# gcorso/DiffDock

Measured on NVIDIA H100. Metric: poses/sec at 20 diffusion steps, higher is better.
Workload: dtype f32

## Files before the change

diffdock_b200/cg_model.py:

```python
from __future__ import annotations

import math
import os

import numpy as np
import torch
from torch import nn

from . import ops
from .irreps import irreps_str, sh_irreps
from .hetero import receptor_blocks
from .layers import (AtomEncoder, GaussianSmearing, _mlp, check_confidence_widths, check_forward, confidence_head, cross_cutoff,
                     cross_graph, edge_cutoff, edge_weight, ligand_graph, score_heads)
from .synthetic import LIG_FEATURE_DIMS as lig_feature_dims, REC_RESIDUE_FEATURE_DIMS as rec_residue_feature_dims
from .tensor_layers import TensorProductConvLayer, get_irrep_seq
from .tp_table import full_tensor_product

_TABLES = os.path.join(os.path.dirname(os.path.abspath(__file__)), 'tables', 'score_norm_tables.npz')
SO3_MIN_EPS, SO3_MAX_EPS, SO3_N_EPS = 0.0005, 4, 2000
TORUS_SIGMA_MIN, TORUS_SIGMA_MAX, TORUS_SIGMA_N = 3e-3, 2, 5000


def _i32(t):
    return t.to(torch.int32).contiguous()
# ... 49 lines not shown
        super().__init__()
        assert parallel == 1, "not implemented"
        unsupported = dict(separate_noise_schedule=separate_noise_schedule,
                           asyncronous_noise_schedule=asyncronous_noise_schedule,
                           include_miscellaneous_atoms=include_miscellaneous_atoms, sidechain_pred=sidechain_pred,
                           depthwise_convolution=depthwise_convolution)
        bad = [k for k, v in unsupported.items() if v]
        if bad:
            raise NotImplementedError(f"{bad}: outside the hot path built so far (SURVEY.md section 8)")
        if lm_embedding_type not in (None, 'precomputed'):
            raise NotImplementedError("on-the-fly ESM embeddings are preprocessing (out of scope); use 'precomputed'")
        self.t_to_sigma, self.device, self.timestep_emb_func = t_to_sigma, device, timestep_emb_func
        self.in_lig_edge_features, self.sigma_embed_dim = in_lig_edge_features, sigma_embed_dim
        self.lig_max_radius, self.rec_max_radius = lig_max_radius, rec_max_radius
        self.cross_max_distance, self.dynamic_max_cross = cross_max_distance, dynamic_max_cross
        self.center_max_distance = center_max_distance
        self.distance_embed_dim, self.cross_distance_embed_dim = distance_embed_dim, cross_distance_embed_dim
        self.sh_lmax = sh_lmax
        self.sh_irreps = irreps_str(sh_irreps(sh_lmax))
        self.ns, self.nv = ns, nv
        self.scale_by_sigma, self.norm_by_sigma = scale_by_sigma, norm_by_sigma
        self.no_torsion, self.smooth_edges, self.odd_parity = no_torsion, smooth_edges, odd_parity
        self.confidence_mode, self.affinity_prediction = confidence_mode, affinity_prediction
        self.atom_confidence, self.atom_num_confidence_outputs = atom_confidence, atom_num_confidence_outputs
        self.num_conv_layers, self.num_prot_emb_layers = num_conv_layers, num_prot_emb_layers
        self.fixed_center_conv, self.no_aminoacid_identities = fixed_center_conv, no_aminoacid_identities
        self.differentiate_convolutions, self.reduce_pseudoscalars = differentiate_convolutions, reduce_pseudoscalars
        self.embed_also_ligand = embed_also_ligand
        self.lm_embedding_type = lm_embedding_type
        lm_dim = 1280 if lm_embedding_type == 'precomputed' else 0
        S, D, Dx = sigma_embed_dim, distance_embed_dim, cross_distance_embed_dim

        self.lig_node_embedding = AtomEncoder(emb_dim=ns, feature_dims=lig_feature_dims, sigma_embed_dim=S)
        self.lig_edge_embedding = _mlp(in_lig_edge_features + S + D, ns, ns, dropout)
        self.rec_node_embedding = AtomEncoder(emb_dim=ns, feature_dims=rec_residue_feature_dims, sigma_embed_dim=0,
                                              lm_embedding_dim=lm_dim)
        self.rec_edge_embedding = _mlp(D, ns, ns, dropout)
        self.rec_sigma_embedding = _mlp(S, ns, ns, dropout)
        self.cross_edge_embedding = _mlp(S + Dx, ns, ns, dropout)
        self.lig_distance_expansion = GaussianSmearing(0.0, lig_max_radius, D)
        self.rec_distance_expansion = GaussianSmearing(0.0, rec_max_radius, D)
        self.cross_distance_expansion = GaussianSmearing(0.0, cross_max_distance, Dx)

        self._irrep_seq = get_irrep_seq(ns, nv, use_second_order_repr, reduce_pseudoscalars)
        self._conv_kw = dict(sh_irreps=self.sh_irreps, n_edge_features=3 * ns, hidden_features=3 * ns, residual=True,
                             batch_norm=batch_norm, dropout=dropout, faster=sh_lmax == 1 and not use_second_order_repr,
                             tp_weights_layers=tp_weights_layers)
        self.rec_emb_layers = nn.ModuleList([self.conv(i, 1) for i in range(num_prot_emb_layers)])
        if embed_also_ligand:
            self.lig_emb_layers = nn.ModuleList([self.conv(i, 1) for i in range(num_prot_emb_layers)])
        self.conv_layers = self._interaction_stack(4, 2)
        self._sync_free = None
        self._prune_receptor = True
        if confidence_mode:
            self._confidence_heads(confidence_dropout, confidence_no_batchnorm, num_confidence_outputs)
            return

        self.center_distance_expansion = GaussianSmearing(0.0, center_max_distance, D)
        self.center_edge_embedding = _mlp(D + S, ns, ns, dropout)
        self.final_conv = TensorProductConvLayer(in_irreps=self.conv_layers[-1].out_irreps, sh_irreps=self.sh_irreps,
                                                 out_irreps='2x1o + 2x1e' if not odd_parity else '1x1o + 1x1e',
                                                 n_edge_features=2 * ns, residual=False, dropout=dropout,
                                                 batch_norm=batch_norm)
        self.tr_final_layer = nn.Sequential(nn.Linear(1 + S, ns), nn.Dropout(dropout), nn.ReLU(), nn.Linear(ns, 1))
        self.rot_final_layer = nn.Sequential(nn.Linear(1 + S, ns), nn.Dropout(dropout), nn.ReLU(), nn.Linear(ns, 1))
        if not no_torsion:
            self.final_edge_embedding = _mlp(D, ns, ns, dropout)
            T, tor_sh = full_tensor_product(self.sh_irreps, '1x2e')
            self.register_buffer('_tor_tp', torch.from_numpy(T).float(), persistent=False)
            self.tor_bond_conv = TensorProductConvLayer(in_irreps=self.conv_layers[-1].out_irreps,
                                                        sh_irreps=irreps_str(tor_sh),
                                                        out_irreps=f'{ns}x0o + {ns}x0e' if not odd_parity else f'{ns}x0o',
                                                        n_edge_features=3 * ns, residual=False, dropout=dropout,
                                                        batch_norm=batch_norm)
            self.tor_final_layer = nn.Sequential(nn.Linear(2 * ns if not odd_parity else ns, ns, bias=False), nn.Tanh(),
                                                 nn.Dropout(dropout), nn.Linear(ns, 1, bias=False))
        z = np.load(_TABLES)
        self.register_buffer('_so3_table', torch.from_numpy(z['so3_exp_score_norms']).float(), persistent=False)
        self.register_buffer('_torus_table', torch.from_numpy(z['torus_score_norm']).float(), persistent=False)

    def _confidence_heads(self, dropout, no_batchnorm, num_confidence_outputs):
        ns = self.ns
        self._conf_tail = (self.nv if self.reduce_pseudoscalars else ns) \
            if self.num_conv_layers + self.num_prot_emb_layers >= 3 else 0
        n_in = ns + self._conf_tail

        def head(i, o):
            bn = (lambda: nn.Identity()) if no_batchnorm else (lambda: nn.BatchNorm1d(ns))
            return nn.Sequential(nn.Linear(i, ns), bn(), nn.ReLU(), nn.Dropout(dropout), nn.Linear(ns, ns), bn(), nn.ReLU(),
                                 nn.Dropout(dropout), nn.Linear(ns, o))
        if self.atom_confidence:
            self.atom_confidence_predictor = head(n_in, self.atom_num_confidence_outputs + ns)
            n_in = ns
        self.confidence_predictor = head(n_in, num_confidence_outputs + (1 if self.affinity_prediction else 0))
        check_confidence_widths(self)

    def conv(self, i, groups):
        seq = self._irrep_seq
        return TensorProductConvLayer(in_irreps=seq[min(i, len(seq) - 1)], out_irreps=seq[min(i + 1, len(seq) - 1)],
                                      edge_groups=groups, **self._conv_kw)

    def _interaction_stack(self, groups, last_groups):
        P, L = self.num_prot_emb_layers, self.num_conv_layers
        return nn.ModuleList([self.conv(i, 1 if not self.differentiate_convolutions else
                                        (last_groups if i == P + L - 1 else groups)) for i in range(P, P + L)])

# ... 105 lines not shown

    def sync_free_crop_capable(self):
        return self.sync_free_capable() and all(layer.fused_capable(self.ns, self.ns) for layer in self.rec_emb_layers)

    @torch.no_grad()
    def forward(self, data):
        check_forward(self, data)
        c = self._static(data)
        if self.sync_free_capable() and max(c['rec_max'], c.get('atom_max', 0)) <= 10000:
            return self._forward_sync_free(data, c)
        if getattr(data, '_crop', None) is not None:
            raise RuntimeError("per-step receptor cropping (data._crop) runs on the sync-free forward only, which this "
                               "batch cannot take (more than 10000 residues in a complex)")
        return self._forward_host_sized(data, c)

    def _interaction_layers(self, node, groups, n_last, merge=False, shared=None, per_layer=None):
        L = len(self.conv_layers)
        for l, layer in enumerate(self.conv_layers):
            use, init = (groups if l < L - 1 else groups[:n_last]), None
            if per_layer is not None and per_layer[1][l] is not None:
                k = per_layer[0]
                use = use[:k] + [per_layer[1][l]] + use[k + 1:]
            if l == 0 and shared is not None:
                init, skip = shared
                use = use[:skip] + [None] + use[skip + 1:]
            if merge:
                use = [tuple(torch.cat([g[k] for g in use]) if use[0][k] is not None else None for k in range(5))]
            node = layer.forward_groups(node, use, gather_scalars=self.ns, init=init)
        return node

    def _forward_sync_free(self, data, c):
        lig, rec = data['ligand'], data['receptor']
        ns, n_lig = self.ns, lig.batch.shape[0]
        tr_sigma, rot_sigma, tor_sigma = self._sigmas(data)

        sig = self.rec_sigma_embedding(self.timestep_emb_func(data.complex_t['tr'])).contiguous()
        crop = getattr(data, '_crop', None)
        prune = self._prune_receptor and len(self.conv_layers) > 1
        keep = None
        if crop is None:
            rec_node, rec_pos = rec.rec_node_attr.clone(), rec.pos.float().contiguous()
            rr_tgt32 = _rr_joint(c, n_lig)
            g_rr = (rr_tgt32[0], rr_tgt32[1], c['rr_ea'], c['rr_vec'], _flat(c['rr_ew']),
                    dict(ea_add=sig, ea_add_idx=c['rr_gid32']))
        else:
            rec_node, rec_pos, g_rr, keep = self._cropped_receptor(data, c, crop, sig, n_lig, select=not prune)
        rec_node[:, :ns] += sig[rec.batch]
        lig_node, g_ll = self._ligand_graph_sync_free(data, c)

        r, rpg = cross_cutoff(self, tr_sigma)
        g_lr, g_rl = self._cross_graph_sync_free(data, c, rec_pos, c['rec_ptr'], c['rec_batch32'],
                                                 c['rec_max'], c['cap_cross'], r, rpg, n_lig, self.cross_edge_embedding,
                                                 self.cross_distance_expansion, vec_sign=-1.0)

        node = torch.cat([lig_node, rec_node], 0)
        groups = [g_ll,
                  g_lr,
                  g_rr,
                  g_rl]
        shared = self._shared_receptor_messages(data, c, rec, rec_node, sig, n_lig) \
            if len(self.conv_layers) > 1 and crop is None else None
        pruned = self._pruned_contact_groups(c, g_rl, keep, sig, n_lig, rec_node.shape[0], shared is not None) \
            if prune else None
        node = self._interaction_layers(node, groups, 2, shared=(shared, 2) if shared is not None else None,
                                        per_layer=(2, pruned) if pruned is not None else None)
        return self._heads(data, c, node[:n_lig], tr_sigma, rot_sigma, tor_sigma, sync_free=True)

    def _need_levels(self, L, shared):
        return [None if l == L - 1 or (l == 0 and shared) else L - 1 - l for l in range(L)]

    def _pruned_contact_groups(self, c, g_rl, keep, sig, n_lig, n_rec, shared):
        levels = self._need_levels(len(self.conv_layers), shared)
        n_levels = max((k for k in levels if k is not None), default=0)
        if n_levels == 0:
            return None
        if 'rr_tgt32l' not in c:
            c['rr_tgt32l'] = (_i32(c['rr_tgt']), _i32(c['rr_src']))
        tgt32, src32 = c['rr_tgt32l']
        key = ('prune', n_lig, n_levels)
        if key not in c:
            c[key] = (torch.empty((n_levels, n_rec), dtype=torch.uint8, device=tgt32.device),
                      [ops.select_edges_buffers(tgt32.shape[0], tgt32.device) for _ in range(n_levels)])
        need_buf, bufs = c[key]
        need = ops.receptor_need(g_rl[0], g_rl[5]['n_edges_dev'], n_lig, tgt32, src32, n_rec, n_levels, keep=keep,
                                 out=need_buf)
        ew, sel = _flat(c['rr_ew']), {}
        for k in sorted({k for k in levels if k is not None}):
            t, s_, perm, gid, n_dev = ops.crop_select_edges(tgt32, src32, keep, c['rr_gid32'], offset=n_lig,
                                                            need=need[k - 1], out=bufs[k - 1])
            sel[k] = (t, s_, c['rr_ea'], c['rr_vec'], ew,
                      dict(n_edges_dev=n_dev, edge_perm=perm, ea_add=sig, ea_add_idx=gid))
        return [sel[k] if k is not None else None for k in levels]

    def _cropped_receptor(self, data, c, crop, sig, n_lig, select=True):
        if not self.sync_free_crop_capable():
            raise RuntimeError("per-step receptor cropping needs every receptor embedding layer on the fused kernel "
                               "(CGModel.sync_free_crop_capable)")
        lig, rec = data['ligand'], data['receptor']
        keep, rec_pos = ops.crop_flags(lig.pos.float().contiguous(), c['lig_ptr'], rec.pos.float().contiguous(),
                                       c['rec_batch32'], crop[0], crop[1])
        if 'rr_tgt32l' not in c:
            c['rr_tgt32l'] = (_i32(c['rr_tgt']), _i32(c['rr_src']))
        if not select and not len(self.rec_emb_layers):
            return rec.rec_node_attr.clone(), rec_pos, None, keep
        tgt, src, perm, gid, n_dev = ops.crop_select_edges(*c['rr_tgt32l'], keep, c['rr_gid32'], offset=n_lig)
        ew = _flat(c['rr_ew'])
# ... 155 lines not shown
```

diffdock_b200/csrc/fused_conv.cu:

```cuda
#include <cuda_bf16.h>
#include <cuda_runtime.h>
#include <stdint.h>
#include <stdlib.h>

#include "../../include/diffdock_b200.h"
#include "sm90.cuh"

namespace {

using namespace ddb200_sm90;

constexpr int BM = 64, BK = 64;
constexpr int CTA_EDGES = 2 * BM;
constexpr int A_KB_BYTES = BM * BK * 2;
constexpr int B_IMAGE_BYTES = 256 * BK * 2;
constexpr int MAX_N = 192;
constexpr int STAGES = 4;
constexpr int STAGE_BYTES = MAX_N * BK * 2;
constexpr int MAX_KB = 5;
constexpr int MAX_KA = MAX_KB;
constexpr int A_IMAGE_BYTES = MAX_KA * A_KB_BYTES;
constexpr int OPS_PER_KB = 8;
constexpr int THREADS = 256;
constexpr int MAX_TILES = 128, MAX_PATHS = 16, MTAB = 48;
constexpr int BAR_WG = 1;
constexpr int SO_STAGES = 3, SO_MAX_PATHS = 32, SO_MTAB = 128;

__device__ __forceinline__ void red_add(float* addr, float v) {
  asm volatile("red.global.add.f32 [%0], %1;" ::"l"(addr), "f"(v) : "memory");
}
__device__ __forceinline__ void wgmma_wait_one() { asm volatile("wgmma.wait_group.sync.aligned 1;" ::: "memory"); }

__device__ __forceinline__ void put_a(unsigned char* sA, int r, int col, __nv_bfloat16 v) {
  const int kb = col >> 6, c = (col & 63) >> 3, j = col & 7;
  *reinterpret_cast<__nv_bfloat16*>(sA + (size_t)kb * A_KB_BYTES + r * 128 + ((c ^ (r & 7)) << 4) + j * 2) = v;
}
__device__ __forceinline__ void put_a2(unsigned char* sA, int r, int col, uint32_t v) {
  const int kb = col >> 6, c = (col & 63) >> 3, j = col & 7;
  *reinterpret_cast<uint32_t*>(sA + (size_t)kb * A_KB_BYTES + r * 128 + ((c ^ (r & 7)) << 4) + j * 2) = v;
}
__device__ __forceinline__ void put_a8(unsigned char* sA, int r, int col0, const uint4& v) {
  const int kb = col0 >> 6, c = (col0 & 63) >> 3;
  *reinterpret_cast<uint4*>(sA + (size_t)kb * A_KB_BYTES + r * 128 + ((c ^ (r & 7)) << 4)) = v;
}
__device__ __forceinline__ void split1(float f, __nv_bfloat16& hi, __nv_bfloat16& lo) {
  hi = __float2bfloat16(f);
  lo = __float2bfloat16(f - __bfloat162float(hi));
}
__device__ __forceinline__ void split8(const float* f, uint4& hi, uint4& lo) {
  uint32_t h[4], l[4];
#pragma unroll
  for (int i = 0; i < 4; ++i) {
    __nv_bfloat16 h0, h1, l0, l1;
    split1(f[2 * i], h0, l0);
    split1(f[2 * i + 1], h1, l1);
    h[i] = (uint32_t)__bfloat16_as_ushort(h0) | ((uint32_t)__bfloat16_as_ushort(h1) << 16);
    l[i] = (uint32_t)__bfloat16_as_ushort(l0) | ((uint32_t)__bfloat16_as_ushort(l1) << 16);
  }
  hi = make_uint4(h[0], h[1], h[2], h[3]);
// ... 651 lines not shown
      atomicAdd(p.dbg + 14, dwait[1]);
      dwait[0] = dwait[1] = 0ull;
    }
  }
  if (p.dbg && blockIdx.x == 0 && tid == 0) {
    unsigned long long g1;
    asm volatile("mov.u64 %0, %%globaltimer;" : "=l"(g1));
    atomicAdd(p.dbg + 25, (unsigned long long)clock64());
    atomicAdd(p.dbg + 26, g1);
  }
}

__global__ void __launch_bounds__(THREADS, 1) fused_conv_kernel(const FusedParams p) { fused_conv_body<false>(p); }
__global__ void __launch_bounds__(THREADS, 1) fused_conv_kernel_so(const FusedParams p) { fused_conv_body<true>(p); }

constexpr int MAX_DEVICES = 64;
struct DeviceState {
  bool attr_done = false, attr_done_so = false;
  bool dbg_init = false;
  unsigned long long* dbg = nullptr;
};
DeviceState g_dev[MAX_DEVICES];

unsigned long long* fused_debug_buffer(int dev) {
  if (dev < 0 || dev >= MAX_DEVICES) return nullptr;
  DeviceState& st = g_dev[dev];
  if (!st.dbg_init) {
    st.dbg_init = true;
    const char* e = getenv("DDB200_FUSED_DEBUG");
    if (e && atoi(e) != 0 && cudaMalloc(&st.dbg, 32 * sizeof(unsigned long long)) == cudaSuccess)
      cudaMemset(st.dbg, 0, 32 * sizeof(unsigned long long));
  }
  return st.dbg;
}

}


extern "C" int ddb200_fused_debug_read(uint64_t* out) {
  int dev = 0;
  cudaGetDevice(&dev);
  unsigned long long* b = fused_debug_buffer(dev);
  if (!b || !out) return DDB200_EINVAL;
  cudaError_t e = cudaDeviceSynchronize();
  if (e == cudaSuccess) e = cudaMemcpy(out, b, 32 * sizeof(unsigned long long), cudaMemcpyDeviceToHost);
  if (e == cudaSuccess) e = cudaMemset(b, 0, 32 * sizeof(unsigned long long));
  return (int)e;
}

namespace {

template <bool SO>
int fused_conv_launch(const ddb200_fused_args* a, void* stream) {
  if (!a || !a->edge_attr || !a->w1_images || !a->w2_images || !a->tiles || !a->mtab || !a->x || !a->edge_vec || !a->sum ||
      !a->tgt || !a->src || a->n_edges < 0 || a->ne <= 0 || a->ns < 0 || a->hidden <= 0 || a->n_tiles <= 0 || a->d_out <= 0)
    return DDB200_EINVAL;
  if (a->ns > 0 && (!a->node || a->ld_node < a->ns)) return DDB200_EINVAL;
  if (a->n_tiles > MAX_TILES || a->n_paths <= 0 || a->n_paths > (SO ? SO_MAX_PATHS : MAX_PATHS) || a->sh_lmax < 0 ||
      a->sh_lmax > 2)
    return DDB200_EINVAL;
  if ((a->ea_add == nullptr) != (a->ea_add_idx == nullptr)) return DDB200_EINVAL;
  const int K1 = a->ne + 2 * a->ns, H = a->hidden;
  const int K1p = (K1 + 15) / 16 * 16, Hp = (H + 15) / 16 * 16;
  const int n_kb = (2 * Hp + 16 + BK - 1) / BK, n_kb1 = (2 * K1p + 16 + BK - 1) / BK;
  if (n_kb > MAX_KB || n_kb1 > MAX_KB || H > MAX_N) return DDB200_EINVAL;
  if ((reinterpret_cast<uintptr_t>(a->w1_images) & 127) || (reinterpret_cast<uintptr_t>(a->w2_images) & 127)) return DDB200_EINVAL;
  if (a->n_hidden < 0 || (a->n_hidden > 0 && (!a->wh_images || (reinterpret_cast<uintptr_t>(a->wh_images) & 127))))
    return DDB200_EINVAL;
  if (a->n_edges == 0) return 0;
  FusedParams p = {};
  p.ea = a->edge_attr; p.ld_ea = a->ld_ea; p.ne = a->ne; p.node = a->node; p.ld_node = a->ld_node; p.ns = a->ns;
  p.tgt = a->tgt; p.src = a->src; p.perm = a->edge_perm; p.ea_add = a->ea_add; p.ea_add_idx = a->ea_add_idx;
  const auto al16 = [](const void* q) { return (reinterpret_cast<uintptr_t>(q) & 15) == 0; };
  p.a0_vec = ((a->ne | a->ns) & 7) == 0 && ((a->ld_ea | (a->ns ? a->ld_node : 0)) & 3) == 0 && al16(a->edge_attr) &&
             (a->ns == 0 || al16(a->node)) && (a->ea_add == nullptr || al16(a->ea_add));
  p.vec_sign = a->vec_sign == 0.f ? 1.f : a->vec_sign;
  p.w1img = reinterpret_cast<const __nv_bfloat16*>(a->w1_images); p.K1 = K1; p.K1p = K1p; p.n_kb1 = n_kb1;
  p.H = H; p.Hp = Hp; p.n_kb = n_kb;
  p.w2img = reinterpret_cast<const __nv_bfloat16*>(a->w2_images); p.tiles = a->tiles; p.n_tiles = a->n_tiles;
  p.whimg = reinterpret_cast<const __nv_bfloat16*>(a->wh_images); p.n_hidden = a->n_hidden;
  p.mtab = a->mtab; p.n_paths = a->n_paths;
  p.x = a->x; p.ld_x = a->ld_x; p.x_vec2 = (a->x_pairs_ok && (a->ld_x & 1) == 0 && (reinterpret_cast<uintptr_t>(a->x) & 7) == 0) ? 1 : 0;
  p.vec = a->edge_vec; p.ew = a->edge_weight; p.lmax = a->sh_lmax; p.sum = a->sum; p.d_out = a->d_out; p.cnt = a->cnt;
  p.n_edges = a->n_edges; p.n_edges_dev = a->n_edges_dev;
  int dev = 0, sms = 132;
  cudaGetDevice(&dev);
  if (dev < 0 || dev >= MAX_DEVICES) return DDB200_EINVAL;
  p.dbg = fused_debug_buffer(dev);
  cudaDeviceGetAttribute(&sms, cudaDevAttrMultiProcessorCount, dev);
  const long long n_mtiles = (a->n_edges + CTA_EDGES - 1) / CTA_EDGES;
  const size_t smem = smem_bytes<SO>();
  if (smem > 227 * 1024) return DDB200_ESMEM;
  auto kernel = SO ? fused_conv_kernel_so : fused_conv_kernel;
  bool& attr_done = SO ? g_dev[dev].attr_done_so : g_dev[dev].attr_done;
  if (!attr_done) {
    const cudaError_t e = cudaFuncSetAttribute(kernel, cudaFuncAttributeMaxDynamicSharedMemorySize, (int)smem);
    if (e != cudaSuccess) return (int)e;
    attr_done = true;
  }
  const unsigned grid = (unsigned)(n_mtiles < sms ? n_mtiles : sms);
  kernel<<<grid, THREADS, smem, (cudaStream_t)stream>>>(p);
  return (int)cudaGetLastError();
}

}

extern "C" int ddb200_fused_conv(const ddb200_fused_args* a, void* stream) { return fused_conv_launch<false>(a, stream); }
// ... 3 lines not shown
```

diffdock_b200/fused.py:

```python
from __future__ import annotations

import ctypes as C
import os

import numpy as np
import torch

from . import _lib
from .ops import PROFILE, _need_cuda, _ptr, _stream

from .irreps import real_cg
from .radial import BK, BN
from .tp_table import TpTable

CONSUMER_KINDS = {(48, 1): (0, 4), (10, 3): (1, 16), (16, 1): (2, 8), (4, 3): (3, 16), (10, 1): (4, 16), (4, 1): (5, 16),
                  (10, 5): (6, 16), (4, 5): (7, 16)}
MAX_K = 144
MAX_TILES = 128
MTAB = 48
MAX_PATHS = 16
MTAB_SO = 128
MAX_PATHS_SO = 32
ENABLED = os.environ.get('DDB200_FUSED_CONV', '1') != '0'

# ... 52 lines not shown
        self.n_hidden = len(hidden)
        self.second_order = second_order(table)
        paths = sorted(table.paths, key=lambda p: (p.i_out, p.w_ref_off))
        tiles, row_src = [], []
        D = 5 if self.second_order else 3
        mtab = np.zeros((len(paths), MTAB_SO if self.second_order else MTAB), dtype=np.float32)
        for pi, p in enumerate(paths):
            C = real_cg(p.l_in, p.l_sh, p.l_out)
            d_in, d_sh, d_out = C.shape
            blk = np.zeros((D, D, 5))
            blk[:d_in, :d_out, :d_sh] = p.coef * np.transpose(C, (0, 2, 1))
            mtab[pi, :D * D * 5] = blk.reshape(-1)
        group_prev = None
        path_prev = None
        for pi, p in enumerate(paths):
            d_in, d_out = 2 * p.l_in + 1, 2 * p.l_out + 1
            kind, rows_per = CONSUMER_KINDS[(p.mul_out, d_out)]
            for u0 in range(0, p.mul_in, rows_per):
                nrow = min(rows_per, p.mul_in - u0)
                n_mma = min(rows_per * p.mul_out, (nrow * p.mul_out + 31) // 32 * 32)
                first = group_prev != p.i_out
                group_prev = p.i_out
                new_path = path_prev is not p
                path_prev = p
                flags = (1 if first else 0) | (4 if new_path else 0) | (p.sh_off << 8)
                tiles.append([kind, n_mma, p.in_off + u0 * d_in, nrow, d_in, p.out_off, flags, pi])
                src = np.full(BN, -1, dtype=np.int64)
                cols = p.w_ref_off + (u0 * p.mul_out) + np.arange(nrow * p.mul_out)
                src[:nrow * p.mul_out] = cols
                row_src.append(src)
        for i in range(len(tiles)):
            if i == len(tiles) - 1 or tiles[i + 1][6] & 1:
                tiles[i][6] |= 2
        self.n_tiles = len(tiles)
        self.n_paths = len(paths)
        src = torch.as_tensor(np.stack(row_src), device=dev)
        ok = src >= 0
        w_rows = torch.zeros((self.n_tiles, BN, H), dtype=torch.float32, device=dev)
        b_rows = torch.zeros((self.n_tiles, BN), dtype=torch.float32, device=dev)
        w_rows[ok] = w2_ref.detach().float()[src[ok]]
        b_rows[ok] = b2_ref.detach().float()[src[ok]]
        self.w2_images = _split_images(w_rows, b_rows, H)
        w1p = torch.zeros((1, BN, K1), dtype=torch.float32, device=dev)
        b1p = torch.zeros((1, BN), dtype=torch.float32, device=dev)
        w1p[0, :H], b1p[0, :H] = w1.detach().float(), b1.detach().float()
        self.w1_images = _split_images(w1p, b1p, K1)
        self.wh_images = None
        if hidden:
            whp = torch.zeros((self.n_hidden, BN, H), dtype=torch.float32, device=dev)
            bhp = torch.zeros((self.n_hidden, BN), dtype=torch.float32, device=dev)
            for l, (w, b) in enumerate(hidden):
                whp[l, :H], bhp[l, :H] = w.detach().float(), b.detach().float()
            self.wh_images = _split_images(whp, bhp, H)
        self.tiles = torch.as_tensor(np.asarray(tiles, dtype=np.int32), device=dev).contiguous()
        self.mtab = torch.as_tensor(mtab, device=dev).contiguous()
        self.x_pairs_ok = int(all(t[2] % 2 == 0 and (t[3] * t[4]) % 2 == 0 for t in tiles))
        s2, s1 = 3 * (_pad16(H) // 16) + 1, 3 * (_pad16(K1) // 16) + 1
        self.mma_flops_per_tile = 2 * 64 * 16 * 192 * (s1 + (self.n_hidden + len(tiles)) * s2)
        self.alg_flops_per_edge = 2 * K1 * H + self.n_hidden * 2 * H * H + 2 * H * table.weight_numel + sum(
            2 * p.mul_in * p.mul_out * (2 * p.l_out + 1) + 2 * p.mul_in * (2 * p.l_in + 1) * (2 * p.l_sh + 1) * (2 * p.l_out + 1)
            for p in table.paths)


class _Args(C.Structure):
    _fields_ = [('edge_attr', C.c_void_p), ('ld_ea', C.c_int64), ('ne', C.c_int32),
                ('node', C.c_void_p), ('ld_node', C.c_int64), ('ns', C.c_int32),
                ('tgt', C.c_void_p), ('src', C.c_void_p), ('edge_perm', C.c_void_p),
                ('ea_add', C.c_void_p), ('ea_add_idx', C.c_void_p), ('vec_sign', C.c_float),
                ('w1_images', C.c_void_p), ('hidden', C.c_int32), ('w2_images', C.c_void_p),
                ('tiles', C.c_void_p), ('n_tiles', C.c_int32), ('mtab', C.c_void_p), ('n_paths', C.c_int32),
                ('x', C.c_void_p), ('ld_x', C.c_int64), ('x_pairs_ok', C.c_int32),
                ('edge_vec', C.c_void_p), ('edge_weight', C.c_void_p), ('sh_lmax', C.c_int32),
                ('n_edges', C.c_int64), ('n_edges_dev', C.c_void_p),
                ('sum', C.c_void_p), ('d_out', C.c_int32), ('cnt', C.c_void_p),
                ('wh_images', C.c_void_p), ('n_hidden', C.c_int32)]


def _p(t):
    return t.data_ptr() if t is not None else None


def fused_conv(plan: FusedPlan, edge_attr, node, ns, tgt32, src32, x, edge_vec, sum_buf, cnt_buf, edge_weight=None,
               edge_perm=None, vec_sign=1.0, ea_add=None, ea_add_idx=None, n_edges_dev=None, n_edges=None):
    _need_cuda(edge_attr, x, edge_vec, sum_buf)
    ne = edge_attr.shape[1]
    E = int(tgt32.shape[0]) if n_edges is None else int(n_edges)
    if E == 0:
        return
    t = plan.table
    assert edge_attr.dtype == torch.float32 and edge_attr.stride(1) == 1 and x.stride(1) == 1 and edge_vec.is_contiguous()
    assert edge_vec.dtype == torch.float32 and x.dtype == torch.float32 and sum_buf.dtype == torch.float32
    assert tgt32.dtype == torch.int32 and src32.dtype == torch.int32 and tgt32.is_contiguous() and src32.is_contiguous()
    assert ne + 2 * ns == plan.k1 and x.shape[1] == t.d_in and sum_buf.shape[1] == t.d_out and sum_buf.is_contiguous()
    if edge_perm is None:
        assert edge_attr.shape[0] >= E and edge_vec.shape[0] >= E
    else:
        assert edge_perm.dtype == torch.int32 and edge_perm.is_contiguous() and edge_perm.shape[0] >= E
    if edge_weight is not None:
        edge_weight = edge_weight.reshape(-1)
        assert edge_weight.dtype == torch.float32 and edge_weight.is_contiguous()
    if ea_add is not None:
        assert ea_add.dtype == torch.float32 and ea_add.is_contiguous() and ea_add.shape[1] == ne
        assert ea_add_idx.dtype == torch.int32 and ea_add_idx.is_contiguous() and ea_add_idx.shape[0] >= E
    if n_edges_dev is not None:
        assert n_edges_dev.dtype == torch.int32 and n_edges_dev.is_cuda
    a = _Args(_p(edge_attr), edge_attr.stride(0), ne, _p(node) if ns else None, node.stride(0) if ns else 0, ns,
              _p(tgt32), _p(src32), _p(edge_perm), _p(ea_add), _p(ea_add_idx) if ea_add is not None else None,
              float(vec_sign), _p(plan.w1_images), plan.hidden, _p(plan.w2_images), _p(plan.tiles), plan.n_tiles,
              _p(plan.mtab), plan.n_paths, _p(x), x.stride(0), plan.x_pairs_ok, _p(edge_vec), _p(edge_weight),
              t.sh_lmax, E, _p(n_edges_dev), _p(sum_buf), t.d_out, _p(cnt_buf), _p(plan.wh_images), plan.n_hidden)
    prof = PROFILE.enabled
    if prof:
        e0, e1 = torch.cuda.Event(enable_timing=True), torch.cuda.Event(enable_timing=True)
        e0.record()
    launch = _lib.lib().ddb200_fused_conv_so if plan.second_order else _lib.lib().ddb200_fused_conv
    rc = launch(C.byref(a), _stream())
    if prof:
        e1.record()
        n_live = int(n_edges_dev.item()) if n_edges_dev is not None else E
        PROFILE.fused_pairs.append((e0, e1))
        PROFILE.fused_bytes += n_live * (4 * t.weight_numel + 12 + 4) + 4 * (sum_buf.shape[0] + 1) + \
            4 * x.shape[0] * t.d_in + 4 * sum_buf.shape[0] * t.d_out
        PROFILE.fused_flops += ((n_live + 63) // 64) * plan.mma_flops_per_tile
        PROFILE.fused_alg_flops += n_live * plan.alg_flops_per_edge
    PROFILE.all_launches += 1
    _lib.check(rc, 'ddb200_fused_conv')
```

include/diffdock_b200.h:

```cpp
#ifndef DIFFDOCK_B200_H
#define DIFFDOCK_B200_H

#include <stddef.h>
#include <stdint.h>

#ifdef __cplusplus
extern "C" {
#endif

#define DDB200_EINVAL (-1)
#define DDB200_ETABLE (-2)
#define DDB200_ESMEM  (-3)

const char* ddb200_version(void);

typedef struct ddb200_tp_table ddb200_tp_table;

int  ddb200_tp_table_create(const int32_t* iblob_host, int n_ints, const float* fblob_host, int n_floats,
                            ddb200_tp_table** out);
void ddb200_tp_table_destroy(ddb200_tp_table* t);
int  ddb200_tp_table_info(const ddb200_tp_table* t, int what);

int ddb200_tpconv_accumulate(const ddb200_tp_table* t, const float* x, int64_t x_stride, const int32_t* edge_src,
                             const int32_t* edge_dst, const float* geo, const float* edge_weight, const float* w,
// ... 16 lines not shown
                       const float* tor_z, const float* coef6, int use_torsion, float* out_pos, void* stream);

int ddb200_pose_update_dev(const float* pos, int64_t n_poses, int n_atoms, int n_bonds, const int32_t* bond_u,
                           const int32_t* bond_v, const uint8_t* mask_rotate, const float* tr_score,
                           const float* rot_score, const float* tor_score, const float* tr_z, const float* rot_z,
                           const float* tor_z, const float* coef_table, const int32_t* step_dev, uint64_t seed,
                           const int64_t* pose_key, int use_torsion, float* out_pos, void* stream);
int ddb200_pose_update_packed(const float* pos, int64_t n_poses, const int32_t* layout, int max_atoms, const int32_t* bond_u,
                              const int32_t* bond_v, const uint8_t* mask_rotate, const float* tr_score,
                              const float* rot_score, const float* tor_score, const float* tr_z, const float* rot_z,
                              const float* tor_z, const float* coef_table, const int32_t* step_dev, uint64_t seed,
                              const int64_t* pose_key, int use_torsion, int32_t* err, float* out_pos, void* stream);
int ddb200_philox_probe(uint64_t seed, int64_t pose_key, uint32_t step, uint32_t block0, int n_blocks,
                        float* out_normals, uint32_t* out_raw, void* stream);

int ddb200_graph_fill(const float* x, const float* y, const int32_t* x_ptr, const int32_t* y_batch,
                      const float* r_per_graph, float r, int64_t n_y, int max_neighbors, int exclude_self,
                      const int32_t* row_start, const int32_t* pre_ptr, const int32_t* pre_col, int32_t* out_row,
                      int32_t* out_col, float* out_vec, int32_t* out_eid, int32_t* slot_out, const int32_t* slot_in,
                      const int32_t* y_ptr, int slot_ld, int32_t* out_perm, int row_offset, int col_offset, void* stream);

int ddb200_csr_sort_by_target(const int32_t* tgt, int64_t n_edges, int32_t n_rows, int32_t* tgt_sorted, int32_t* perm,
                              int32_t* row_ptr, void* workspace, size_t* workspace_bytes, void* stream);

int ddb200_edge_embed(const float* edge_vec, const int32_t* edge_row, const float* u, const float* w1_rbf, const float* w2,
                      const float* b2, int rbf_dim, int ns, const float* rbf_offset, float rbf_coeff, int64_t capacity,
                      const int32_t* n_edges_dev, float* out, void* stream);

int ddb200_radial_gemm(const float* h, int64_t ldh, int64_t n_edges, int K, const void* b_images, const float* bias,
                       int n_tiles_n, float* out, int64_t ldo, void* stream);

int ddb200_radial_mlp(const float* edge_attr, int64_t ld_ea, int ne, const float* node, int64_t ld_node, int ns,
                      const int32_t* tgt, const int32_t* src, const void* w1_images, const float* b1, int hidden,
                      const void* w2_images, const float* b2, int n_tiles_n, int64_t n_edges, float* out, int64_t ldo,
                      void* stream);

typedef struct ddb200_fused_args {
  const float*   edge_attr;   int64_t ld_ea;   int32_t ne;
  const float*   node;        int64_t ld_node; int32_t ns;
  const int32_t* tgt;         const int32_t* src;
  const int32_t* edge_perm;
  const float*   ea_add;      const int32_t* ea_add_idx;
  float          vec_sign;
  const void*    w1_images;   int32_t hidden;
  const void*    w2_images;
  const int32_t* tiles;       int32_t n_tiles;
  const float*   mtab;        int32_t n_paths;
  const float*   x;           int64_t ld_x;    int32_t x_pairs_ok;
  const float*   edge_vec;    const float* edge_weight;
  int32_t        sh_lmax;
  int64_t        n_edges;     const int32_t* n_edges_dev;
  float*         sum;         int32_t d_out;   float* cnt;
  const void*    wh_images;   int32_t n_hidden;
} ddb200_fused_args;

int ddb200_fused_conv(const ddb200_fused_args* args, void* stream);
int ddb200_fused_conv_so(const ddb200_fused_args* args, void* stream);

int ddb200_fused_debug_read(uint64_t* out);

int ddb200_contact_count(const float* pos, int32_t n, float cutoff, int32_t max_neighbors, int32_t knn_only,
                         int32_t* count, void* stream);
int ddb200_contact_fill(const float* pos, int32_t n, float cutoff, int32_t max_neighbors, int32_t knn_only,
                        const int32_t* row_start, int32_t* out_nbr, int32_t* out_ctr, void* stream);

int ddb200_crop_flags(const float* lig_pos, const int32_t* lig_ptr, const float* rec_pos, const int32_t* rec_batch,
                      int64_t n_rec, const float* cutoff2_table, const int32_t* step_dev, uint8_t* keep,
                      float* rec_pos_masked, void* stream);
int ddb200_crop_select_edges(const int32_t* tgt, const int32_t* src, const int32_t* gid, int64_t n_edges,
                             const uint8_t* keep, const uint8_t* need, int32_t offset, int32_t* out_tgt, int32_t* out_src,
                             int32_t* out_perm, int32_t* out_gid, int32_t* n_selected, void* workspace,
                             size_t* workspace_bytes, void* stream);
int ddb200_receptor_need(const int32_t* cross_tgt, const int32_t* n_cross, int64_t cross_cap, int32_t offset,
                         const int32_t* tgt, const int32_t* src, int64_t n_edges, const uint8_t* keep, int64_t n_rec,
                         int32_t n_levels, uint8_t* need, void* stream);

#define DDB200_CONF_MAX_IN 256
#define DDB200_CONF_MAX_HIDDEN 128
#define DDB200_CONF_MAX_OUT 16
int ddb200_confidence_head(const float* x, int64_t ld_x, int64_t n_cols, const int32_t* lig_ptr, int32_t n_poses,
                           int32_t n_head, int32_t tail_off, int32_t n_tail, const float* atom_mlp, int32_t atom_hidden,
                           int32_t n_atom_out, const float* mlp, int32_t n_in, int32_t n_hidden, int32_t n_out,
                           float* confidence, float* atom_confidence, void* stream);

#ifdef __cplusplus
}
#endif
#endif
```

Baseline: 23.85.

## Add per-target reduce path for ligand-receptor cross-edge convolution

Adds a new three-kernel path for the ligand-to-receptor cross convolution. It computes the per-edge hidden layer, reduces edges per target before applying the second radial weight layer (using split-bf16 wgmma), and then contracts with w2 per target instead of per edge. This reassociation is meant to avoid materializing per-edge tensor-product weights when many edges share a target. In exchange it adds a large workspace buffer, extra launches and a sorted-target assumption, and it only runs when the plan qualifies (n_zcols at least 512, path limits met).

```diff
diff --git a/diffdock_b200/cg_model.py b/diffdock_b200/cg_model.py
--- a/diffdock_b200/cg_model.py
+++ b/diffdock_b200/cg_model.py
@@ -125,6 +125,7 @@
         self.conv_layers = self._interaction_stack(4, 2)
         self._sync_free = None
         self._prune_receptor = True
+        self._lig_rec_reduce = True
         if confidence_mode:
             self._confidence_heads(confidence_dropout, confidence_no_batchnorm, num_confidence_outputs)
             return
@@ -336,6 +337,8 @@
         g_lr, g_rl = self._cross_graph_sync_free(data, c, rec_pos, c['rec_ptr'], c['rec_batch32'],
                                                  c['rec_max'], c['cap_cross'], r, rpg, n_lig, self.cross_edge_embedding,
                                                  self.cross_distance_expansion, vec_sign=-1.0)
+        if self._lig_rec_reduce:
+            g_lr[5]['n_targets'] = n_lig
 
         node = torch.cat([lig_node, rec_node], 0)
         groups = [g_ll,
diff --git a/diffdock_b200/csrc/fused_conv.cu b/diffdock_b200/csrc/fused_conv.cu
--- a/diffdock_b200/csrc/fused_conv.cu
+++ b/diffdock_b200/csrc/fused_conv.cu
@@ -5,6 +5,8 @@
 
 #include "../../include/diffdock_b200.h"
 #include "sm90.cuh"
+
+int lig_rec_reduce_launch(const ddb200_fused_args* a, void* stream);
 
 namespace {
 
@@ -762,7 +764,8 @@
 
 template <bool SO>
 int fused_conv_launch(const ddb200_fused_args* a, void* stream) {
-  if (!a || !a->edge_attr || !a->w1_images || !a->w2_images || !a->tiles || !a->mtab || !a->x || !a->edge_vec || !a->sum ||
+  if (a && a->mode != 0) return (!SO && a->mode == 1) ? lig_rec_reduce_launch(a, stream) : DDB200_EINVAL;
+  if (!a ||!a->edge_attr || !a->w1_images || !a->w2_images || !a->tiles || !a->mtab || !a->x || !a->edge_vec || !a->sum ||
       !a->tgt || !a->src || a->n_edges < 0 || a->ne <= 0 || a->ns < 0 || a->hidden <= 0 || a->n_tiles <= 0 || a->d_out <= 0)
     return DDB200_EINVAL;
   if (a->ns > 0 && (!a->node || a->ld_node < a->ns)) return DDB200_EINVAL;
diff --git a/diffdock_b200/csrc/lig_rec_reduce.cu b/diffdock_b200/csrc/lig_rec_reduce.cu
--- /dev/null
+++ b/diffdock_b200/csrc/lig_rec_reduce.cu
@@ -0,0 +1,384 @@
+#include <cuda_bf16.h>
+#include <cuda_runtime.h>
+#include <stdint.h>
+
+#include "../../include/diffdock_b200.h"
+#include "sm90.cuh"
+
+namespace {
+
+using namespace ddb200_sm90;
+
+constexpr int THREADS = 256;
+constexpr int HMAX = 144;
+constexpr int KMAX = 144;
+constexpr int HE = 128, HLD = HE + 4, HKC = 32;
+constexpr int KE = 64, ZB = 128, MAX_PATHS = 16, MAX_PP = 10, BN_ROWS = 160;
+constexpr int A_BYTES = ZB * 128, B_BYTES = BN_ROWS * 128;
+constexpr int OT = 64, OLD = OT + 4, MAX_UD = 144, MAX_UW = 48 * 48;
+
+struct LrParams {
+  const float* ea; long long ld_ea; int ne;
+  const float* node; long long ld_node; int ns;
+  const int* tgt; const int* src; const int* perm;
+  const float* ea_add; const int* ea_add_idx;
+  float vec_sign;
+  const float* x; long long ld_x;
+  const float* vec; const float* ew;
+  long long n_edges; const int* n_edges_dev;
+  float* sum; int d_out; float* cnt;
+  const float* w1; const float* b1; const float* w2t; int H, K1;
+  const float* mtab; const int* paths; int n_paths; const int* cols; int n_cols, n_cb;
+  float* hbuf; float* pbuf;
+};
+
+__device__ __forceinline__ long long live_edges(const LrParams& p) {
+  long long n = p.n_edges;
+  if (p.n_edges_dev) { const long long nd = __ldg(p.n_edges_dev); n = nd < n ? (nd < 0 ? 0 : nd) : n; }
+  return n;
+}
+
+__device__ __forceinline__ long long lower_bound(const int* __restrict__ a, long long n, int v) {
+  long long lo = 0, hi = n;
+  while (lo < hi) {
+    const long long mid = (lo + hi) >> 1;
+    if (__ldg(a + mid) < v) lo = mid + 1; else hi = mid;
+  }
+  return lo;
+}
+
+__global__ void __launch_bounds__(THREADS, 2) lr_hidden_kernel(const LrParams p) {
+  extern __shared__ __align__(16) float smem[];
+  float* sA = smem;
+  float* sW = sA + KMAX * HLD;
+  const long long n = live_edges(p);
+  const long long e0 = (long long)blockIdx.x * HE;
+  if (e0 >= n) return;
+  const int tid = threadIdx.x, K1 = p.K1, H = p.H;
+  {
+    const int r = tid >> 1, part = tid & 1;
+    const long long e = e0 + r;
+    const bool live = e < n;
+    const long long er = (live && p.perm) ? (long long)__ldg(p.perm + e) : e;
+    const float* ea_row = p.ea + er * p.ld_ea;
+    const float* add_row = (live && p.ea_add) ? p.ea_add + (long long)__ldg(p.ea_add_idx + e) * p.ne : nullptr;
+    const float* t_row = p.ns ? p.node + (long long)(live ? __ldg(p.tgt + e) : 0) * p.ld_node - p.ne : nullptr;
+    const float* s_row = p.ns ? p.node + (long long)(live ? __ldg(p.src + e) : 0) * p.ld_node - p.ne - p.ns : nullptr;
+    for (int k0 = part; k0 < K1; k0 += 16) {
+      float v[8];
+#pragma unroll
+      for (int j = 0; j < 8; ++j) {
+        const int k = k0 + 2 * j;
+        v[j] = 0.f;
+        if (live && k < K1) {
+          if (k < p.ne) v[j] = __ldg(ea_row + k) + (add_row ? __ldg(add_row + k) : 0.f);
+          else v[j] = __ldg((k < p.ne + p.ns ? t_row : s_row) + k);
+        }
+      }
+#pragma unroll
+      for (int j = 0; j < 8; ++j)
+        if (k0 + 2 * j < K1) sA[(k0 + 2 * j) * HLD + r] = v[j];
+    }
+  }
+  const int th = tid & 15, te = tid >> 4;
+  float acc[8][9];
+#pragma unroll
+  for (int r = 0; r < 8; ++r)
+#pragma unroll
+    for (int j = 0; j < 9; ++j) acc[r][j] = 0.f;
+  for (int kc = 0; kc < K1; kc += HKC) {
+    __syncthreads();
+    for (int idx = tid; idx < HKC * HMAX; idx += THREADS) {
+      const int h = idx / HKC, kk = idx - h * HKC;
+      sW[kk * HMAX + h] = (h < H && kc + kk < K1) ? __ldg(p.w1 + (long long)h * K1 + kc + kk) : 0.f;
+    }
+    __syncthreads();
+    const int kn = min(HKC, K1 - kc);
+#pragma unroll 2
+    for (int kk = 0; kk < kn; ++kk) {
+      const float4 a0 = *reinterpret_cast<const float4*>(sA + (kc + kk) * HLD + 8 * te);
+      const float4 a1 = *reinterpret_cast<const float4*>(sA + (kc + kk) * HLD + 8 * te + 4);
+      const float av[8] = {a0.x, a0.y, a0.z, a0.w, a1.x, a1.y, a1.z, a1.w};
+#pragma unroll
+      for (int j = 0; j < 9; ++j) {
+        const float wv = sW[kk * HMAX + th + 16 * j];
+#pragma unroll
+        for (int r = 0; r < 8; ++r) acc[r][j] = fmaf(av[r], wv, acc[r][j]);
+      }
+    }
+  }
+#pragma unroll
+  for (int j = 0; j < 9; ++j) {
+    const int h = th + 16 * j;
+    const float b = h < H ? __ldg(p.b1 + h) : 0.f;
+#pragma unroll
+    for (int r = 0; r < 8; ++r) {
+      const long long e = e0 + 8 * te + r;
+      if (e < n) p.hbuf[e * HMAX + h] = h < H ? fmaxf(acc[r][j] + b, 0.f) : 0.f;
+    }
+  }
+}
+
+__device__ __forceinline__ void put_pair(unsigned char* img, int r, int k, float a, float b, unsigned char* img_lo) {
+  const __nv_bfloat16 ha = __float2bfloat16(a), hb = __float2bfloat16(b);
+  const __nv_bfloat16 la = __float2bfloat16(a - __bfloat162float(ha)), lb = __float2bfloat16(b - __bfloat162float(hb));
+  const uint32_t off = r * 128 + (((k >> 3) ^ (r & 7)) << 4) + (k & 7) * 2;
+  __nv_bfloat162 h2, l2;
+  h2.x = ha; h2.y = hb; l2.x = la; l2.y = lb;
+  *reinterpret_cast<__nv_bfloat162*>(img + off) = h2;
+  *reinterpret_cast<__nv_bfloat162*>(img_lo + off) = l2;
+}
+
+__global__ void __launch_bounds__(THREADS, 2) lr_reduce_kernel(const LrParams p, int t0) {
+  extern __shared__ __align__(1024) unsigned char smem_raw[];
+  unsigned char* base = smem_raw + ((1024 - (smem_u32(smem_raw) & 1023)) & 1023);
+  unsigned char* sA = base;
+  unsigned char* sB = sA + 2 * A_BYTES;
+  float* sM = reinterpret_cast<float*>(sB + 2 * B_BYTES);
+  float* sY = sM + KE * MAX_PP * 9;
+  int4* sCol = reinterpret_cast<int4*>(sY + KE * 9);
+  int* sSrc = reinterpret_cast<int*>(sCol + ZB);
+  __shared__ long long sRange[2];
+  const int tid = threadIdx.x, wg = tid >> 7, t128 = tid & 127, H = p.H;
+  const int cb = blockIdx.x, tl = blockIdx.y, t = t0 + tl;
+  const long long n = live_edges(p);
+  if (tid < 2) sRange[tid] = lower_bound(p.tgt, n, t + tid);
+  const int c0 = cb * ZB;
+  const int p_lo = __ldg(p.cols + 4 * c0 + 2), p_hi = __ldg(p.cols + 4 * (min(c0 + ZB, p.n_cols) - 1) + 2);
+  const int npp = p_hi - p_lo + 1;
+  if (tid < ZB) {
+    const int c = c0 + tid;
+    sCol[tid] = c < p.n_cols ? __ldg(reinterpret_cast<const int4*>(p.cols) + c) : make_int4(0, 0, -1, 0);
+  }
+  __syncthreads();
+  const int beg = (int)sRange[0], end = (int)sRange[1];
+  if (cb == 0 && tid == 0 && p.cnt && end > beg) atomicAdd(p.cnt + t, (float)(end - beg));
+
+  float d[80];
+#pragma unroll
+  for (int i = 0; i < 80; ++i) d[i] = 0.f;
+  const uint32_t a_desc = gmma_desc_lo(smem_u32(sA + wg * 64 * 128));
+  const uint32_t b_desc = gmma_desc_lo(smem_u32(sB));
+  for (int e0 = beg; e0 < end; e0 += KE) {
+    const int ne = min(KE, end - e0);
+    __syncthreads();
+    if (tid < KE) {
+      const bool vb = tid < ne;
+      const int eb = e0 + tid;
+      const long long erb = (vb && p.perm) ? (long long)__ldg(p.perm + eb) : eb;
+      const float ew_b = (vb && p.ew) ? __ldg(p.ew + erb) : 1.f;
+      float vx = vb ? p.vec_sign * __ldg(p.vec + 3 * erb) : 1.f, vy = vb ? p.vec_sign * __ldg(p.vec + 3 * erb + 1) : 0.f,
+            vz = vb ? p.vec_sign * __ldg(p.vec + 3 * erb + 2) : 0.f;
+      const float nrm = fmaxf(sqrtf(vx * vx + vy * vy + vz * vz), 1e-12f);
+      vx /= nrm; vy /= nrm; vz /= nrm;
+      const float s3 = 1.7320508075688772f, s5 = 2.23606797749979f, s15 = 3.872983346207417f;
+      float* Y = sY + tid * 9;
+      Y[0] = ew_b;
+      Y[1] = ew_b * (s3 * vx); Y[2] = ew_b * (s3 * vy); Y[3] = ew_b * (s3 * vz);
+      Y[4] = ew_b * (s15 * vx * vz);
+      Y[5] = ew_b * (s15 * vx * vy);
+      Y[6] = ew_b * (s5 * (vy * vy - 0.5f * (vx * vx + vz * vz)));
+      Y[7] = ew_b * (s15 * vy * vz);
+      Y[8] = ew_b * (0.5f * s15 * (vz * vz - vx * vx));
+      sSrc[tid] = vb ? __ldg(p.src + eb) : 0;
+    }
+#pragma unroll 1
+    for (int idx = tid; idx < BN_ROWS * (KE / 2); idx += THREADS) {
+      const int h = idx % BN_ROWS, kp = idx / BN_ROWS, i = 2 * kp;
+      float a = 0.f, b = 0.f;
+      if (h < H) {
+        if (i < ne) a = p.hbuf[(long long)(e0 + i) * HMAX + h];
+        if (i + 1 < ne) b = p.hbuf[(long long)(e0 + i + 1) * HMAX + h];
+      } else if (h == H) {
+        a = i < ne ? 1.f : 0.f;
+        b = i + 1 < ne ? 1.f : 0.f;
+      }
+      put_pair(sB, h, i, a, b, sB + B_BYTES);
+    }
+    __syncthreads();
+#pragma unroll 1
+    for (int idx = tid; idx < KE * npp * 9; idx += THREADS) {
+      const int i = idx / (npp * 9), r = idx - i * npp * 9, pp = r / 9, ik = r - pp * 9;
+      const int* pi = p.paths + 12 * (p_lo + pp);
+      const int sh_off = __ldg(pi + 8);
+      const float* T = p.mtab + 48 * __ldg(pi + 9) + ik * 5;
+      const float* Y = sY + i * 9;
+      float a = 0.f;
+#pragma unroll
+      for (int j = 0; j < 5; ++j) a = fmaf(__ldg(T + j), Y[min(sh_off + j, 8)], a);
+      sM[(i * MAX_PP + pp) * 9 + ik] = a;
+    }
+    __syncthreads();
+    {
+      constexpr int IT = 2;
+      const int c = tid & (ZB - 1);
+      const int4 ci = sCol[c];
+#pragma unroll 1
+      for (int kp0 = tid / ZB; kp0 < KE / 2; kp0 += 2 * IT) {
+        float xv[IT][2][3];
+#pragma unroll
+        for (int it = 0; it < IT; ++it)
+#pragma unroll
+          for (int q = 0; q < 2; ++q) {
+            const int i = 2 * (kp0 + 2 * it) + q;
+            xv[it][q][0] = xv[it][q][1] = xv[it][q][2] = 0.f;
+            if (i < ne && ci.z >= 0) {
+              const float* xr = p.x + (long long)sSrc[i] * p.ld_x + ci.x;
+              xv[it][q][0] = __ldg(xr);
+              if (ci.y == 3) { xv[it][q][1] = __ldg(xr + 1); xv[it][q][2] = __ldg(xr + 2); }
+            }
+          }
+#pragma unroll
+        for (int it = 0; it < IT; ++it) {
+          float v[2];
+#pragma unroll
+          for (int q = 0; q < 2; ++q) {
+            const int i = 2 * (kp0 + 2 * it) + q;
+            v[q] = 0.f;
+            if (i < ne && ci.z >= 0) {
+              const float* M = sM + (i * MAX_PP + (ci.z - p_lo)) * 9;
+              const int k = ci.w;
+              if (ci.y == 1) v[q] = xv[it][q][0] * M[k];
+              else v[q] = fmaf(xv[it][q][2], M[6 + k], fmaf(xv[it][q][1], M[3 + k], xv[it][q][0] * M[k]));
+            }
+          }
+          put_pair(sA, c, 2 * (kp0 + 2 * it), v[0], v[1], sA + A_BYTES);
+        }
+      }
+    }
+    fence_proxy_async();
+    __syncthreads();
+    wgmma_fence_regs(d);
+    wgmma_fence();
+#pragma unroll
+    for (int st = 0; st < KE / 16; ++st) {
+      const uint64_t ahi = gmma_desc(a_desc + 2 * st), alo = gmma_desc(a_desc + (A_BYTES >> 4) + 2 * st);
+      const uint64_t bhi = gmma_desc(b_desc + 2 * st), blo = gmma_desc(b_desc + (B_BYTES >> 4) + 2 * st);
+      Wgmma<BN_ROWS>::mma(d, ahi, bhi, 1u);
+      Wgmma<BN_ROWS>::mma(d, ahi, blo, 1u);
+      Wgmma<BN_ROWS>::mma(d, alo, bhi, 1u);
+    }
+    wgmma_commit();
+    wgmma_wait_all();
+    wgmma_fence_regs(d);
+  }
+  const long long zp = (long long)p.n_cb * ZB;
+  float* P = p.pbuf + (long long)tl * (H + 1) * zp + c0 + 64 * wg + 16 * (t128 >> 5) + ((t128 & 31) >> 2);
+  const int q2 = 2 * (t128 & 3);
+#pragma unroll
+  for (int j = 0; j < BN_ROWS / 8; ++j) {
+#pragma unroll
+    for (int b = 0; b < 2; ++b) {
+      const int h = 8 * j + q2 + b;
+      if (h <= H) {
+        P[h * zp] = d[4 * j + b];
+        P[h * zp + 8] = d[4 * j + 2 + b];
+      }
+    }
+  }
+}
+
+__global__ void __launch_bounds__(THREADS) lr_out_kernel(const LrParams p, int t0, int nt) {
+  __shared__ __align__(16) float sA[MAX_UD * OLD];
+  __shared__ float sB[MAX_UW];
+  const int tid = threadIdx.x, H = p.H;
+  const int* pi = p.paths + 12 * blockIdx.y;
+  const int U = __ldg(pi), W = __ldg(pi + 1), D = __ldg(pi + 2), zoff = __ldg(pi + 3), woff = __ldg(pi + 4),
+            out_off = __ldg(pi + 5), ld_w2t = __ldg(pi + 10);
+  const int OP = W * D, UD = U * D, UW = U * W, ng = min(8, THREADS / OP);
+  const int o = tid % OP, g = tid / OP, w = o / D, k = o - w * D;
+  const int tb = blockIdx.x * OT;
+  const long long zp = (long long)p.n_cb * ZB;
+  float acc[2][8];
+#pragma unroll
+  for (int s = 0; s < 2; ++s)
+#pragma unroll
+    for (int j = 0; j < 8; ++j) acc[s][j] = 0.f;
+  for (int h = 0; h <= H; ++h) {
+    __syncthreads();
+    for (int idx = tid; idx < UD * OT; idx += THREADS) {
+      const int tt = idx / UD, j = idx - tt * UD;
+      sA[j * OLD + tt] = tb + tt < nt ? p.pbuf[((long long)(tb + tt) * (H + 1) + h) * zp + zoff + j] : 0.f;
+    }
+    for (int idx = tid; idx < UW; idx += THREADS) sB[idx] = __ldg(p.w2t + (long long)h * ld_w2t + woff + idx);
+    __syncthreads();
+    if (g < ng) {
+      for (int u = 0; u < U; ++u) {
+        const float b = sB[u * W + w];
+        const float* a = sA + (u * D + k) * OLD;
+#pragma unroll
+        for (int s = 0; s < 2; ++s) {
+          const int gg = g + s * ng;
+          if (gg < 8) {
+            const float4 a0 = *reinterpret_cast<const float4*>(a + 8 * gg);
+            const float4 a1 = *reinterpret_cast<const float4*>(a + 8 * gg + 4);
+            acc[s][0] = fmaf(a0.x, b, acc[s][0]); acc[s][1] = fmaf(a0.y, b, acc[s][1]);
+            acc[s][2] = fmaf(a0.z, b, acc[s][2]); acc[s][3] = fmaf(a0.w, b, acc[s][3]);
+            acc[s][4] = fmaf(a1.x, b, acc[s][4]); acc[s][5] = fmaf(a1.y, b, acc[s][5]);
+            acc[s][6] = fmaf(a1.z, b, acc[s][6]); acc[s][7] = fmaf(a1.w, b, acc[s][7]);
+          }
+        }
+      }
+    }
+  }
+  if (g >= ng) return;
+#pragma unroll
+  for (int s = 0; s < 2; ++s) {
+    const int gg = g + s * ng;
+    if (gg >= 8) continue;
+#pragma unroll
+    for (int j = 0; j < 8; ++j) {
+      const int tt = tb + 8 * gg + j;
+      if (tt < nt) atomicAdd(p.sum + (long long)(t0 + tt) * p.d_out + out_off + o, acc[s][j]);
+    }
+  }
+}
+
+constexpr size_t HIDDEN_SMEM = (size_t)(KMAX * HLD + HKC * HMAX) * 4;
+constexpr size_t REDUCE_SMEM = 2 * (size_t)(A_BYTES + B_BYTES) + (size_t)(KE * MAX_PP * 9 + KE * 9) * 4 + ZB * 16 + KE * 4 + 1024;
+
+constexpr int MAX_DEVICES = 64;
+bool g_attr_done[MAX_DEVICES];
+
+}
+
+int lig_rec_reduce_launch(const ddb200_fused_args* a, void* stream) {
+  if (!a->edge_attr || !a->x || !a->edge_vec || !a->sum || !a->tgt || !a->src || !a->mtab || !a->work || !a->w1f ||
+      !a->b1f || !a->w2t || !a->lr_paths || !a->lr_cols || a->n_edges < 0 || a->ne <= 0 || a->ns < 0 || a->hidden <= 0 ||
+      a->hidden > HMAX || a->ne + 2 * a->ns > KMAX || a->n_paths <= 0 || a->n_paths > MAX_PATHS || a->n_zcols <= 0 ||
+      a->n_targets < 0 || a->chunk_targets <= 0 || a->d_out <= 0 || a->n_hidden != 0 || a->sh_lmax < 0 || a->sh_lmax > 2)
+    return DDB200_EINVAL;
+  if (a->ns > 0 && (!a->node || a->ld_node < a->ns)) return DDB200_EINVAL;
+  if ((a->ea_add == nullptr) != (a->ea_add_idx == nullptr)) return DDB200_EINVAL;
+  if (a->n_edges == 0 || a->n_targets == 0) return 0;
+  LrParams p = {};
+  p.ea = a->edge_attr; p.ld_ea = a->ld_ea; p.ne = a->ne; p.node = a->node; p.ld_node = a->ld_node; p.ns = a->ns;
+  p.tgt = a->tgt; p.src = a->src; p.perm = a->edge_perm; p.ea_add = a->ea_add; p.ea_add_idx = a->ea_add_idx;
+  p.vec_sign = a->vec_sign == 0.f ? 1.f : a->vec_sign;
+  p.x = a->x; p.ld_x = a->ld_x; p.vec = a->edge_vec; p.ew = a->edge_weight;
+  p.n_edges = a->n_edges; p.n_edges_dev = a->n_edges_dev;
+  p.sum = a->sum; p.d_out = a->d_out; p.cnt = a->cnt;
+  p.w1 = a->w1f; p.b1 = a->b1f; p.w2t = a->w2t; p.H = a->hidden; p.K1 = a->ne + 2 * a->ns;
+  p.mtab = a->mtab; p.paths = a->lr_paths; p.n_paths = a->n_paths; p.cols = a->lr_cols; p.n_cols = a->n_zcols;
+  p.n_cb = (a->n_zcols + ZB - 1) / ZB;
+  p.hbuf = a->work;
+  p.pbuf = a->work + a->n_edges * (long long)HMAX;
+  int dev = 0;
+  cudaGetDevice(&dev);
+  if (dev < 0 || dev >= MAX_DEVICES) return DDB200_EINVAL;
+  if (!g_attr_done[dev]) {
+    cudaError_t e = cudaFuncSetAttribute(lr_hidden_kernel, cudaFuncAttributeMaxDynamicSharedMemorySize, (int)HIDDEN_SMEM);
+    if (e == cudaSuccess)
+      e = cudaFuncSetAttribute(lr_reduce_kernel, cudaFuncAttributeMaxDynamicSharedMemorySize, (int)REDUCE_SMEM);
+    if (e != cudaSuccess) return (int)e;
+    g_attr_done[dev] = true;
+  }
+  const cudaStream_t s = (cudaStream_t)stream;
+  lr_hidden_kernel<<<(unsigned)((a->n_edges + HE - 1) / HE), THREADS, HIDDEN_SMEM, s>>>(p);
+  for (int t0 = 0; t0 < a->n_targets; t0 += a->chunk_targets) {
+    const int nt = a->n_targets - t0 < a->chunk_targets ? a->n_targets - t0 : a->chunk_targets;
+    lr_reduce_kernel<<<dim3((unsigned)p.n_cb, (unsigned)nt), THREADS, REDUCE_SMEM, s>>>(p, t0);
+    lr_out_kernel<<<dim3((unsigned)((nt + OT - 1) / OT), (unsigned)a->n_paths), THREADS, 0, s>>>(p, t0, nt);
+  }
+  return (int)cudaGetLastError();
+}
diff --git a/diffdock_b200/fused.py b/diffdock_b200/fused.py
--- a/diffdock_b200/fused.py
+++ b/diffdock_b200/fused.py
@@ -128,6 +128,25 @@
             for l, (w, b) in enumerate(hidden):
                 whp[l, :H], bhp[l, :H] = w.detach().float(), b.detach().float()
             self.wh_images = _split_images(whp, bhp, H)
+        self.lr_paths = None
+        if not self.second_order and not hidden and all(
+                p.mul_out * (2 * p.l_out + 1) <= 48 and p.mul_in * (2 * p.l_out + 1) <= 144 and p.mul_in * p.mul_out <= 2304
+                for p in paths):
+            lp, cols, z = [], [], 0
+            for pi, p in enumerate(paths):
+                d_in, d_out = 2 * p.l_in + 1, 2 * p.l_out + 1
+                lp.append([p.mul_in, p.mul_out, d_out, z, p.w_ref_off, p.out_off, d_in, p.in_off, p.sh_off, pi,
+                           table.weight_numel, 0])
+                cols += [[p.in_off + u * d_in, d_in, pi, k] for u in range(p.mul_in) for k in range(d_out)]
+                z += p.mul_in * d_out
+            cp = [c[2] for c in cols]
+            if max(cp[min(c0 + LR_ZB, z) - 1] - cp[c0] + 1 for c0 in range(0, z, LR_ZB)) <= LR_MAX_PP:
+                self.lr_paths = torch.as_tensor(np.asarray(lp, dtype=np.int32), device=dev).contiguous()
+                self.lr_cols = torch.as_tensor(np.asarray(cols, dtype=np.int32), device=dev).contiguous()
+                self.n_zcols = z
+                self.w1f = w1.detach().float().contiguous()
+                self.b1f = b1.detach().float().contiguous()
+                self.w2t = torch.cat([w2_ref.detach().float().t(), b2_ref.detach().float()[None]], 0).contiguous()
         self.tiles = torch.as_tensor(np.asarray(tiles, dtype=np.int32), device=dev).contiguous()
         self.mtab = torch.as_tensor(mtab, device=dev).contiguous()
         self.x_pairs_ok = int(all(t[2] % 2 == 0 and (t[3] * t[4]) % 2 == 0 for t in tiles))
@@ -149,7 +168,19 @@
                 ('edge_vec', C.c_void_p), ('edge_weight', C.c_void_p), ('sh_lmax', C.c_int32),
                 ('n_edges', C.c_int64), ('n_edges_dev', C.c_void_p),
                 ('sum', C.c_void_p), ('d_out', C.c_int32), ('cnt', C.c_void_p),
-                ('wh_images', C.c_void_p), ('n_hidden', C.c_int32)]
+                ('wh_images', C.c_void_p), ('n_hidden', C.c_int32),
+                ('mode', C.c_int32), ('n_targets', C.c_int32), ('work', C.c_void_p), ('chunk_targets', C.c_int32),
+                ('w1f', C.c_void_p), ('b1f', C.c_void_p), ('w2t', C.c_void_p),
+                ('lr_paths', C.c_void_p), ('lr_cols', C.c_void_p), ('n_zcols', C.c_int32)]
+
+
+LR_P_BUDGET = 1 << 30
+LR_H_BUDGET = 4 << 30
+LR_ZB = 128
+LR_MAX_PP = 10
+LR_MAX_CHUNK = 65535
+LR_LAUNCHES = 0
+LR_MIN_ZCOLS = 512
 
 
 def _p(t):
@@ -157,7 +188,7 @@
 
 
 def fused_conv(plan: FusedPlan, edge_attr, node, ns, tgt32, src32, x, edge_vec, sum_buf, cnt_buf, edge_weight=None,
-               edge_perm=None, vec_sign=1.0, ea_add=None, ea_add_idx=None, n_edges_dev=None, n_edges=None):
+               edge_perm=None, vec_sign=1.0, ea_add=None, ea_add_idx=None, n_edges_dev=None, n_edges=None, n_targets=None):
     _need_cuda(edge_attr, x, edge_vec, sum_buf)
     ne = edge_attr.shape[1]
     E = int(tgt32.shape[0]) if n_edges is None else int(n_edges)
@@ -185,6 +216,20 @@
               float(vec_sign), _p(plan.w1_images), plan.hidden, _p(plan.w2_images), _p(plan.tiles), plan.n_tiles,
               _p(plan.mtab), plan.n_paths, _p(x), x.stride(0), plan.x_pairs_ok, _p(edge_vec), _p(edge_weight),
               t.sh_lmax, E, _p(n_edges_dev), _p(sum_buf), t.d_out, _p(cnt_buf), _p(plan.wh_images), plan.n_hidden)
+    reduce = False
+    if n_targets is not None and plan.lr_paths is not None and plan.n_zcols >= LR_MIN_ZCOLS and \
+            0 < n_targets <= sum_buf.shape[0]:
+        zp = -(-plan.n_zcols // LR_ZB) * LR_ZB
+        per_target = (plan.hidden + 1) * zp
+        chunk = min(int(n_targets), LR_MAX_CHUNK, max(1, LR_P_BUDGET // (4 * per_target)))
+        reduce = 4 * E * MAX_K <= LR_H_BUDGET
+    if reduce:
+        global LR_LAUNCHES
+        LR_LAUNCHES += 1
+        work = torch.empty(E * MAX_K + chunk * per_target, dtype=torch.float32, device=sum_buf.device)
+        a.mode, a.n_targets, a.work, a.chunk_targets = 1, int(n_targets), work.data_ptr(), chunk
+        a.w1f, a.b1f, a.w2t = _p(plan.w1f), _p(plan.b1f), _p(plan.w2t)
+        a.lr_paths, a.lr_cols, a.n_zcols = _p(plan.lr_paths), _p(plan.lr_cols), plan.n_zcols
     prof = PROFILE.enabled
     if prof:
         e0, e1 = torch.cuda.Event(enable_timing=True), torch.cuda.Event(enable_timing=True)
@@ -197,7 +242,11 @@
         PROFILE.fused_pairs.append((e0, e1))
         PROFILE.fused_bytes += n_live * (4 * t.weight_numel + 12 + 4) + 4 * (sum_buf.shape[0] + 1) + \
             4 * x.shape[0] * t.d_in + 4 * sum_buf.shape[0] * t.d_out
-        PROFILE.fused_flops += ((n_live + 63) // 64) * plan.mma_flops_per_tile
+        if not reduce:
+            PROFILE.fused_flops += ((n_live + 63) // 64) * plan.mma_flops_per_tile
+        else:
+            chunks = int(((torch.bincount(tgt32[:n_live].long(), minlength=n_targets)[:n_targets] + 63) // 64).sum())
+            PROFILE.fused_flops += chunks * (-(-plan.n_zcols // LR_ZB)) * 2 * 12 * 2 * 64 * 160 * 16
         PROFILE.fused_alg_flops += n_live * plan.alg_flops_per_edge
     PROFILE.all_launches += 1
     _lib.check(rc, 'ddb200_fused_conv')
diff --git a/include/diffdock_b200.h b/include/diffdock_b200.h
--- a/include/diffdock_b200.h
+++ b/include/diffdock_b200.h
@@ -92,6 +92,10 @@
   int64_t        n_edges;     const int32_t* n_edges_dev;
   float*         sum;         int32_t d_out;   float* cnt;
   const void*    wh_images;   int32_t n_hidden;
+  int32_t        mode;        int32_t n_targets;
+  float*         work;        int32_t chunk_targets;
+  const float*   w1f;         const float* b1f;   const float* w2t;
+  const int32_t* lr_paths;    const int32_t* lr_cols;  int32_t n_zcols;
 } ddb200_fused_args;
 
 int ddb200_fused_conv(const ddb200_fused_args* args, void* stream);
```

Measured after the change: 24.87, median of 6. 1.04x the previous value.
